# Chunyu-Hugh/SymbolicRegression.jl

Measured on AMD Instinct MI355X. Metric: tree-node x row evals/sec (batched eval_loss, fp32), higher is better.
Workload: dtype f32

## Files before the change

symbolicregression.jl_amd/csrc/sr_capi.cpp:

```cpp
#include <hip/hip_runtime.h>
#include <rccl/rccl.h>
#include <dlfcn.h>
#include <limits.h>
#include <stdlib.h>

#include <algorithm>
#include <atomic>
#include <chrono>
#include <cmath>
#include <cstdio>
#include <cstdlib>
#include <cstring>
#include <deque>
#include <functional>
#include <memory>
#include <mutex>
#include <string>
#include <vector>

#include "../../include/sr_amd.h"
#include "sr_compile.h"
#include "sr_eval.h"
#include "sr_fold.h"
#include "sr_fold_dev.h"
// ... 206 lines not shown
  DevBuf stamps;
  int64_t n_stamps = 0;
#endif
  std::unique_ptr<SrComm> xport;
  int comm_ranks = 0;
  int comm_rank = 0;
  uint64_t comm_gen = 0;
  DevBuf coll_buf, coll_packed, ctl;
  HostBuf h_coll;
  double last_eval_ms = 0.0, last_total_ms = 0.0;
  double last_busy_ms = 0.0;
  bool timing_pending = false;
  double phase_ms[5] = {0, 0, 0, 0, 0};
  std::chrono::steady_clock::time_point phase_t;
  void start_phases(std::chrono::steady_clock::time_point t) {
    phase_t = t;
    for (double& v : phase_ms) v = 0.0;
  }
  void mark_phase(int i) {
    const auto now = std::chrono::steady_clock::now();
    phase_ms[i] = std::chrono::duration<double, std::milli>(now - phase_t).count();
    phase_t = now;
  }
  int cu_count = 256;
  std::vector<uint32_t> perm_host;
  DevBuf fold_cand;
  DevBuf fold_list;
  DevBuf fold_wg;
  DevBuf loss_list;
  DevBuf fold_est;
  DevBuf fold_dbg;
  DevBuf fold_code, fold_tab, fold_store, fold_ctl, fold_io2, fold_sq, fold_tab2;
  std::shared_ptr<void> fold_job;
  size_t outs_fval_off = 0, outs_fst_off = 0, outs_bytes_all = 0;
  hipEvent_t ev_fc0[kMaxChunks] = {}, ev_fc1[kMaxChunks] = {};
  int64_t n_ref_ok_last = 0, n_ref_fail_last = 0;
  double fold_kernel_ms_last = 0.0;
// ... 297 lines not shown

template <typename T>
struct BatchCall {
  sr_ctx* ctx;
  const EvalReq& req;
  const BatchWants& want;
  SrProgramBatch<T>* prog;
  BatchResult* res;
  sr_ctx::LastCall scratch;
  sr_ctx::LastCall& last;
  bool allow_derived;
  BatchCall(sr_ctx* c, const EvalReq& q, const BatchWants& w, SrProgramBatch<T>* p, BatchResult* r)
      : ctx(c), req(q), want(w), prog(p), res(r), last(w.internal ? scratch : c->last), allow_derived(w.allow_derived) {}
  void mark_phase(int i) {
    if (!want.internal) ctx->mark_phase(i);
  }
  bool gather = false, multi = false;
  int64_t n_eval = 0, n_rows_up = 0, nt = 0, total_nodes = 0;
  int mrb = 0, lkind = 0;
  double lparam = 0.0;
  const sr_ctx::LossExpr* lexpr = nullptr;
  const sr_param_batch* pb = nullptr;
  bool parametric = false;
  int nfk = 0;
  int64_t p_stride = 0;
  double max_abs_p = 0.0;
  int tier = 0, R = 0, W = 0, Rv = 0, n_rb = 1, n_chunks = 1;
  SrBuildRequest breq;
  GridSpec gs;
  Grid g_ls, g_vs;
// ... 117 lines not shown
    img = sr_prog_image(total_nodes, nt, sizeof(SrIns<T>), multi ? size_t(req.views->n_views) : 0);
    SR_HIP_CHECK(ctx->prog.ensure(img.bytes));
    SR_HIP_CHECK(ctx->h_prog.ensure(img.bytes, s, ctx->stream2));
    dprog = ctx->prog.as<char>();
    ctx->d_code = dprog;
    ctx->d_off = reinterpret_cast<uint32_t*>(dprog + img.o_off);
    ctx->d_bad = reinterpret_cast<uint8_t*>(dprog + img.o_bad);
    ctx->d_perm = reinterpret_cast<uint32_t*>(dprog + img.o_perm);
    ctx->d_end = reinterpret_cast<uint32_t*>(dprog + img.o_end);
    n_part = size_t(nt) * size_t(n_rb);
    SR_HIP_CHECK(ctx->part_sum.ensure(n_part * sizeof(double) + 8));
    SR_HIP_CHECK(ctx->part_flag.ensure(n_part * sizeof(uint32_t) + 4));
    return SR_OK;
  }

  int plan_fold() {
    fold_n_terms = want.shard ? ((req.ds->w && req.ds->shard_w_min < 0.0) ? 0 : want.n_total)
                              : fold_terms(req.ds, n_eval, req.loss_kind);
    if (want.shard) ctx->fold_job.reset();
    if (want.fold && ctx->ref_fold && want.mode == SR_MODE_LOSS && nt > 0 && fold_n_terms > 0) {
      FoldPlanIn in;
      in.nt = nt;
      in.n_eval = n_eval;
      in.max_shard = want.shard ? sr_max_shard_rows(req.ds->shard_offs, n_eval) : n_eval;
      in.fold_len = want.shard ? want.n_total : n_eval;
      in.elem_size = int(sizeof(T));
      in.tier = tier;
      in.R = R;
      in.Rv = Rv;
      in.fold_store_mb = ctx->fold_store_mb;
      in.fold_slot_mb = ctx->fold_slot_mb;
      in.fold_seg_max = ctx->fold_seg_max;
      in.fold_rows_max = ctx->fold_rows_max;
      in.g_ls = g_ls;
      in.g_vs = g_vs;
      in.g_big = gs.over(in.max_shard, std::max<int64_t>(512, (in.max_shard + ctx->fold_seg_max - 1) /
                                                                     std::max<int64_t>(1, ctx->fold_seg_max)))
                     .grid(nt, R, 1);
      fold = sr_fold_plan(in);
      if (fold.path == 1) {
        SR_HIP_CHECK(ctx->fold_store.ensure(size_t(nt) * size_t(fold.pos_rows) * sizeof(T)));
      } else if (fold.path == 2) {
        SR_HIP_CHECK(ctx->fold_store.ensure(size_t(fold.slots) * size_t(fold.slot_rows) * sizeof(T)));
        SR_HIP_CHECK(ctx->fold_ctl.ensure(64));
        SR_HIP_CHECK(hipMemsetAsync(ctx->fold_ctl.p, 0, 4 * sizeof(int), s));
      }
      if (fold.path && ctx->fold_stats) {
        SR_HIP_CHECK(ctx->fold_dbg.ensure(size_t(nt) * sizeof(int4) + 16));
        SR_HIP_CHECK(hipMemsetAsync(ctx->fold_dbg.p, 0, size_t(nt) * sizeof(int4), s));
      }
      if (fold.path) {
        SR_HIP_CHECK(ctx->fold_code.ensure(n_part * sizeof(int32_t) + 4));
        SR_HIP_CHECK(ctx->fold_tab.ensure(n_part * sizeof(typename SrFoldTab<T>::Pair) + 16));
        SR_HIP_CHECK(ctx->fold_sq.ensure(n_part * sizeof(int32_t) + 4));
        SR_HIP_CHECK(ctx->fold_tab2.ensure(n_part * sizeof(typename SrFoldTab<T>::Pair) + 16));
      }
    }
    fold_cand = fold.path == 2 && ctx->fold_single_pass && sizeof(T) == 4 && tier == SR_TIER_BASIC && !gather &&
                !multi && !want.shard && !parametric && n_rb > 1;
    if (fold_cand) SR_HIP_CHECK(ctx->fold_cand.ensure(n_part * sizeof(int4) + 16));
    if (fold_cand && ctx->fold_cand_est) {
      SR_HIP_CHECK(ctx->fold_est.ensure(size_t(nt) * (sizeof(double) + sizeof(uint32_t)) + 8));
      SR_HIP_CHECK(hipMemsetAsync(ctx->fold_est.p, 0, size_t(nt) * (sizeof(double) + sizeof(uint32_t)), s));
    }
    fold_compact = fold.path == 2 && ctx->fold_compact && !gather && !multi && !want.shard && !parametric;
    if (fold_compact) {
      SR_HIP_CHECK(ctx->fold_list.ensure(n_part * sizeof(int32_t) + 4));
      SR_HIP_CHECK(ctx->fold_wg.ensure(sr_fold_wg_words(n_rb) * sizeof(int32_t)));
    }
    loss_compact = fold_compact && fold_cand && ctx->loss_compact && want.mode == SR_MODE_LOSS;
    if (loss_compact) SR_HIP_CHECK(ctx->loss_list.ensure(sr_loss_list_bytes(nt)));
    for (int c = 0; c < kMaxChunks; ++c) last.loss_listed_np[c] = 0;
    last.loss_list_nt = nt;
    last.loss_list_read = true;
    last.n_loss_listed_launches = last.n_loss_live = last.n_loss_excl = 0;
    for (int r = 0; r < 2 * kMaxChunks; ++r) {
      last.fold_wg_nrb[r] = 0;
      for (int k = 0; k < 4; ++k) last.fold_wg_info[r][k] = 0.0;
    }
    last.fold_wg_read = true;
    last.fold_path = res->fold_path = fold.path;
    last.fold_timed = false;
    last.fold_cand_read = fold.path != 2;
    last.n_cand_taken = last.n_cand_rerun = 0;
    return SR_OK;
// ... 103 lines not shown
    ctx->h_perm_last = h_perm;
    h_end = reinterpret_cast<uint32_t*>(hprog + img.o_end);
    last.n_chunks = 0;
    last.derived = false;
    last.n_derived = 0;
    last.timed = ctx->timing != 0 && !want.internal;
    if (last.timed) SR_HIP_CHECK(hipEventRecord(ctx->ev_start, s));
    if (gather)
      SR_HIP_CHECK(hipMemcpyAsync(ctx->row_idx.p, req.row_idx, size_t(n_rows_up) * sizeof(int64_t), hipMemcpyHostToDevice,
                                  s));
    if (parametric && nt > 0 && p_stride > 0)
      SR_HIP_CHECK(hipMemcpyAsync(ctx->ptab.p, ctx->h_ptab.p, size_t(nt) * size_t(p_stride) * sizeof(T), hipMemcpyHostToDevice, s));
    return SR_OK;
  }

  int launch_derived() {
    dld = (n_eval + kRowAlign - 1) / kRowAlign * kRowAlign;
    max_abs_x = leaf_bound(want.shard ? want.shard->max_abs_x : req.ds->max_abs_x);
    const int64_t derived_rows = want.shard ? want.shard->min_rows : n_eval;
    if (allow_derived && ctx->derived && want.mode == SR_MODE_LOSS && tier == SR_TIER_BASIC &&
        derived_rows >= kDerivedMinRows && nt >= 64 && double(nt) * double(derived_rows) >= kDerivedMinWork &&
        max_abs_x < double(tbig())) {
      choose_derived(*req.trees, ctx->opsets[req.opset_id], req.ds->nf, &spec, &dmap);
      if (spec.n > 0) {
        SR_HIP_CHECK(ctx->derived_cols.ensure(size_t(spec.n) * size_t(dld) * sizeof(T)));
        if (last.timed) SR_HIP_CHECK(hipEventRecord(ctx->ev_d0, s));
        SR_HIP_CHECK(sr_launch_derived<T>(static_cast<const T*>(req.ds->X), req.ds->ld,
                                          gather ? ctx->row_idx.as<int64_t>() : nullptr, n_eval, dld, spec,
                                          ctx->derived_cols.as<T>(), dld, s));
        if (last.timed) SR_HIP_CHECK(hipEventRecord(ctx->ev_d1, s));
        last.derived = true;
        last.n_derived = spec.n;
      } else {
        dmap.clear();
      }
    }
    stress_probe = use_probe && !gather && req.ds->probe_rows != nullptr && ctx->stress_probe;
    if (stress_probe && !dmap.empty()) {
      SR_HIP_CHECK(ctx->probe_derived.ensure(size_t(spec.n) * size_t(kProbeRows) * sizeof(T)));
      SR_HIP_CHECK(sr_launch_derived<T>(static_cast<const T*>(req.ds->X), req.ds->ld,
                                        static_cast<const int64_t*>(req.ds->probe_rows), req.ds->n_probe, kProbeRows, spec,
                                        ctx->probe_derived.as<T>(), kProbeRows, s));
    }
    return SR_OK;
  }

  int begin_chunks() {
    if (n_chunks > 1) {
      SR_HIP_CHECK(ctx->need_stream2());
      SR_HIP_CHECK(hipEventRecord(ctx->ev_join, s));
// ... 7 lines not shown
    fjob.slot_rows = fold.slot_rows;
    fjob.n_terms = fold_n_terms;
    fjob.delta = std::ldexp(1.0, -ctx->fold_delta_log2);
    fjob.fuse_reduce = fold.path == 1 && !want.shard && want.mode == SR_MODE_LOSS;
    fjob.slot_cap = fold.path == 2
                        ? int(std::min<int64_t>({int64_t(INT_MAX / 2), fold.slot_budget,
                                                 int64_t(ctx->fold_store.cap / (size_t(fold.slot_rows) * sizeof(T)))}))
                        : 0;
    char* const outs_base = (host_out || fold_mirror) ? ctx->h_outs.as<char>() : ctx->outs.as<char>();
    d_fval = reinterpret_cast<T*>(outs_base + ctx->outs_fval_off);
    d_fst = reinterpret_cast<int32_t*>(outs_base + ctx->outs_fst_off);
    t_pre = std::chrono::steady_clock::now();
    return SR_OK;
  }

  int compile_chunk(BatchChunk<T>& ch) {
    static const bool phase_debug = std::getenv("SR_AMD_PHASE_DEBUG") != nullptr;
    const int64_t t0 = ch.t0 = cplan.bound[ch.c];
    const int64_t nc = ch.nc = cplan.bound[ch.c + 1] - t0;
    for (int64_t t = t0; t < t0 + nc; ++t)
      ch.max_nodes = std::max<uint32_t>(ch.max_nodes, uint32_t(req.trees->offsets[t + 1] - req.trees->offsets[t]));
    ch.cs = (ch.c & 1) ? ctx->stream2 : s;
    sr_tree_batch sub = *req.trees;
    sub.n_trees = nc;
    sub.offsets = req.trees->offsets + t0;
    ch.pc.keep_pieces = true;
    const SrParamNodes pnodes{parametric ? pb->is_parameter : nullptr, parametric ? pb->parameter : nullptr,
                              parametric ? pb->max_parameters : 0};
    const int rc = sr_compile_batch<T>(sub, ctx->opsets[req.opset_id], want.n_total, req.ds->nf, false, &ch.pc, &err,
                                       dmap.empty() ? nullptr : dmap.data(), parametric ? &pnodes : nullptr);
    if (rc != SR_OK) {
      if (rc == SR_ERR_BAD_TREE || rc == SR_ERR_INVALID_ARG) {
        const size_t at = err.find("tree ");
        if (at == 0) {
          const int64_t k = std::atoll(err.c_str() + 5);
          err = "tree " + std::to_string(k + t0) + err.substr(err.find(':'));
        }
      }
      return set_error(rc, err);
    }
    if (ch.c == 0) {
      if (phase_debug) {
        const auto now = std::chrono::steady_clock::now();
        std::fprintf(stderr, "[sr phase] trees %lld chunks %d: setup %.3f ms, compile of chunk 0 (%lld trees) %.3f ms\n",
                     (long long)nt, n_chunks, std::chrono::duration<double, std::milli>(t_pre - ctx->phase_t).count(),
                     (long long)nc, std::chrono::duration<double, std::milli>(now - t_pre).count());
      }
      mark_phase(0);
    }
    ch.depth = ch.pc.max_depth > 0 ? ch.pc.max_depth : 1;
    ch.ncode = ch.pc.n_code;
    return SR_OK;
  }

  int order_and_stage(BatchChunk<T>& ch) {
    const SrProgramBatch<T>& pc = ch.pc;
    const int64_t t0 = ch.t0, nc = ch.nc;
    ch.n_vs = sr_count_vstk(pc.depth.data(), nc, Rv > 0);
    if (ch.n_vs > 0) ch.g_vs = gs.grid(ch.n_vs, Rv, 0);
// ... 240 lines not shown
      who.mflag = reinterpret_cast<uint32_t*>(ctx->h_outs.as<char>() + ctx->outs_flag_off);
    }
    for (const FoldRegion<T>& fr : fjob.regions) {
      SR_STAGE(fold_steps<T>(ctx, fjob, fr, who, cs));
      SR_STAGE(fold_walk<T>(ctx, fjob, fr, who, nullptr, d_fval, d_fst, cs));
    }
    fjob.regions.clear();
    if (last.timed) {
      SR_HIP_CHECK(hipEventRecord(ctx->ev_fc1[ch.c], cs));
      last.fold_timed = true;
    }
    return SR_OK;
  }

  int run_chunk(int c) {
    BatchChunk<T> ch;
    ch.c = c;
    SR_STAGE(compile_chunk(ch));
    SR_STAGE(order_and_stage(ch));
    SR_STAGE(upload_chunk(ch));
    if (last.timed) SR_HIP_CHECK(hipEventRecord(ctx->ev_c0[c], ch.cs));
    if (ch.n_vs > 0) SR_STAGE(launch_region(ch, 0, ch.n_vs, true));
    if (ch.n_vs < ch.nc) SR_STAGE(launch_region(ch, ch.n_vs, ch.nc - ch.n_vs, false));
    if (last.timed) SR_HIP_CHECK(hipEventRecord(ctx->ev_c1[c], ch.cs));
    if (early) SR_HIP_CHECK(hipEventRecord(ctx->ev_red[c], ch.cs));
    if (early && c == n_chunks - 1) {
      for (int k = 0; k < c; ++k) SR_HIP_CHECK(hipStreamWaitEvent(ch.cs, ctx->ev_red[k], 0));
      SR_HIP_CHECK(hipMemcpyAsync(ctx->h_outs.as<char>() + ctx->outs_flag_off, ctx->outs.as<char>() + ctx->outs_flag_off,
                                  size_t(nt) * sizeof(uint32_t), hipMemcpyDeviceToHost, ch.cs));
      SR_HIP_CHECK(hipEventRecord(ctx->ev_flags, ch.cs));
    }
    if (fold.path && !want.shard && !fjob.regions.empty()) SR_STAGE(fold_chunk(ch));
    last.n_chunks = c + 1;
    code_base += uint32_t(ch.ncode);
    return SR_OK;
  }

  int run() {
    SR_STAGE(validate_call());
    SR_STAGE(stage_param_table());
    choose_kernels();
    SR_STAGE(bind_buffers());
    in_flight = true;
    SR_STAGE(plan_fold());
    SR_STAGE(plan_chunks());
    SR_STAGE(bind_outputs());
    SR_STAGE(prepare_hints());
    SR_STAGE(begin_programs());
    SR_STAGE(launch_derived());
    SR_STAGE(begin_chunks());
    for (int c = 0; c < n_chunks && nt > 0; ++c) SR_STAGE(run_chunk(c));
    if (n_chunks > 1) {
      SR_HIP_CHECK(hipEventRecord(ctx->ev_join, ctx->stream2));
      SR_HIP_CHECK(hipStreamWaitEvent(s, ctx->ev_join, 0));
    }
    if (nt == 0) mark_phase(0);
    res->grid = glast;
    if (fold.path && want.shard) ctx->fold_job = std::make_shared<FoldJob<T>>(std::move(fjob));
    mark_phase(1);
    return SR_OK;
  }
};

template <typename T>
// ... 765 lines not shown
        float km = 0.f;
        if (hipEventElapsedTime(&km, ctx->ev_k0, ctx->ev_k1) == hipSuccess) ctx->exact_kernel_ms += double(km);
      }
      exact_done = one_batch || mc == 0;
      return SR_OK;
    }();
    if (rc != SR_OK) {
      (void)hipStreamSynchronize(s);
      if (ctx->stream2) (void)hipStreamSynchronize(ctx->stream2);
      if (ctx->stream3) (void)hipStreamSynchronize(ctx->stream3);
      return rc;
    }
  } else {
    SR_HIP_CHECK(hipStreamSynchronize(s));
  }
  if (!ctx->host_reductions.empty()) host_reduce_partials(ctx, nt);
  std::vector<double> sums(hs, hs + nt);
  std::vector<uint32_t> flags(hf, hf + nt);
  ctx->timing_pending = true;
  if (!c.res.early) {
    ctx->mark_phase(2);
    big_list(flags.data(), &list);
    list_ok.assign(list.size(), 1);
    ctx->n_exact_last = int64_t(list.size());
    ctx->exact_kernel_ms = 0.0;
  }
  for (int v = 0; v < n_views && !list.empty() && !exact_done; ++v) {
    std::vector<int64_t> lv;
    std::vector<size_t> at;
    for (size_t i = 0; i < list.size(); ++i)
// ... 62 lines not shown
  ctx->n_fold_last = int64_t(fold_list.size());
  ctx->fold_slow_last = ctx->fold_seg_last = 0;
  for (double& v : ctx->fold_ms) v = 0.0;
  for (int v = 0; v < n_views && !fold_list.empty(); ++v) {
    std::vector<int64_t> fv;
    for (int64_t t : fold_list)
      if (view_of(t) == v) fv.push_back(t);
    if (fv.empty()) continue;
    std::vector<T> fold;
    rc = fold_exact<T>(ctx, q.view(v), n_eval, fv, &fold);
    if (rc != SR_OK) return rc;
    const T den = (ds->w && n_eval > 0) ? jl_wsum_view<T>(ds, rows_of(v), n_eval) : T(vden[size_t(v)]);
    for (size_t i = 0; i < fv.size(); ++i) static_cast<T*>(c.out_loss)[fv[i]] = T(fold[i] / den);
  }
  ctx->mark_phase(4);
  auto t1 = std::chrono::steady_clock::now();
  ctx->last_total_ms = std::chrono::duration<double, std::milli>(t1 - c.t0).count();
  return SR_OK;
}

template <typename T>
int eval_loss_impl(sr_ctx* ctx, const EvalReq& req, void* out_loss, uint8_t* out_complete) {
  LossCall<T> c;
  const int rc = eval_loss_submit<T>(ctx, req, out_loss, out_complete, &c);
  if (rc != SR_OK) return rc;
  return eval_loss_finish<T>(ctx, c);
}

template <typename T>
int eval_pred_impl(sr_ctx* ctx, const EvalReq& req, void* out_pred, uint8_t* out_complete) {
// ... 2102 lines not shown
      int64_t entries = 0, longest = 0;
      for (int b = 0; b < nrb; ++b) {
        entries += cnt[b];
        longest = std::max<int64_t>(longest, cnt[b]);
      }
      ctx->last.fold_wg_info[r][0] = double(wg0[nrb]);
      ctx->last.fold_wg_info[r][1] = double(entries);
      ctx->last.fold_wg_info[r][2] = double(wg0[nrb + 1]);
      ctx->last.fold_wg_info[r][3] = double(longest);
    }
    ctx->last.fold_wg_read = true;
  }
  for (int r = 0; r < 2 * kMaxChunks; ++r)
    for (int k = 0; k < 4; ++k)
      if (n > 19 + 4 * r + k) out[19 + 4 * r + k] = ctx->last.fold_wg_info[r][k];
  return SR_OK;
}

int sr_set_tuning(sr_ctx* ctx, const char* name, int64_t value) {
  if (check_ctx(ctx) != SR_OK) return SR_ERR_INVALID_ARG;
  if (!name) return set_error(SR_ERR_INVALID_ARG, "tuning knob name is NULL");
  Lock l(ctx);
  std::string err;
  return sr_knob_set(*ctx, name, value, &err) == 0 ? SR_OK : set_error(SR_ERR_INVALID_ARG, err);
}

int sr_last_grad_info(sr_ctx* ctx, int n, double* kernel_ms, double* flops, int64_t* items, int* rows_per_lane) {
  if (check_ctx(ctx) != SR_OK) return SR_ERR_INVALID_ARG;
  Lock l(ctx);
  for (int b = 0; b < n && b < sr_ctx::kGradBuckets; ++b) {
// ... 69 lines not shown
```

symbolicregression.jl_amd/csrc/sr_compile.cpp:

```cpp
#include "sr_compile.h"

#include <unistd.h>

#include <algorithm>
#include <atomic>
#include <chrono>
#include <cstdlib>
#include <cmath>
#include <condition_variable>
#include <cstring>
#include <functional>
#include <mutex>
#include <thread>

namespace {

class WorkerPool {
 public:
  static WorkerPool& get() {
    static std::mutex m;
    static WorkerPool* pool = nullptr;
    std::lock_guard<std::mutex> g(m);
    if (!pool || pool->pid_ != getpid()) pool = new WorkerPool();
    return *pool;
  }
  int size() const { return int(threads_.size()) + 1; }
  void run(int n, const std::function<void(int)>& fn) {
    std::lock_guard<std::mutex> batch(batch_mu_);
    uint64_t g;
    {
      std::lock_guard<std::mutex> lk(mu_);
      g = ++gen_;
      job_ = &fn;
      n_jobs_ = n;
      done_.store(0);
      ticket_.store(g << 32);
      gen_pub_.store(g, std::memory_order_release);
    }
    if (n > 1 && !threads_.empty()) cv_.notify_all();
    drain(g, &fn, n);
    while (done_.load(std::memory_order_acquire) < n) std::this_thread::yield();
  }

 private:
  WorkerPool() : pid_(getpid()) {
    unsigned hc = std::thread::hardware_concurrency();
    int n = int(hc == 0 ? 4 : (hc > 16 ? 16 : hc));
    if (const char* v = std::getenv("SR_AMD_COMPILE_THREADS")) n = std::atoi(v) > 0 ? std::atoi(v) : 1;
    if (const char* v = std::getenv("SR_AMD_COMPILE_SPIN_US")) spin_us_ = std::max(0, std::atoi(v));
    --n;
    for (int i = 0; i < n; ++i) threads_.emplace_back([this] { loop(); });
    for (auto& t : threads_) t.detach();
  }
  void drain(uint64_t g, const std::function<void(int)>* job, int n) {
    uint64_t t = ticket_.load();
    for (;;) {
      if ((t >> 32) != g || int(t & 0xffffffffu) >= n) return;
      if (!ticket_.compare_exchange_weak(t, t + 1)) continue;
      (*job)(int(t & 0xffffffffu));
      done_.fetch_add(1, std::memory_order_release);
      t = ticket_.load();
    }
  }
  void loop() {
    uint64_t seen = 0;
    for (;;) {
      uint64_t g;
      const std::function<void(int)>* job;
      int n;
      const auto t0 = std::chrono::steady_clock::now();
      while (gen_pub_.load(std::memory_order_acquire) == seen &&
             std::chrono::steady_clock::now() - t0 < std::chrono::microseconds(spin_us_))
        std::this_thread::yield();
      {
        std::unique_lock<std::mutex> lk(mu_);
        cv_.wait(lk, [&] { return gen_ != seen; });
        seen = g = gen_;
        job = job_;
        n = n_jobs_;
      }
      drain(g, job, n);
    }
  }
  pid_t pid_;
  std::vector<std::thread> threads_;
  std::mutex batch_mu_, mu_;
  std::condition_variable cv_;
  const std::function<void(int)>* job_ = nullptr;
  int n_jobs_ = 0;
  std::atomic<uint64_t> ticket_{0};
  std::atomic<int> done_{0};
  uint64_t gen_ = 0;
  std::atomic<uint64_t> gen_pub_{0};
  int spin_us_ = 0;
};

struct NameId {
  const char* name;
  uint32_t id;
};

const NameId kUnary[] = {
    {"neg", SR_U_NEG},       {"-", SR_U_NEG},          {"square", SR_U_SQUARE},  {"cube", SR_U_CUBE},
    {"exp", SR_U_EXP},       {"cos", SR_U_COS},        {"sin", SR_U_SIN},        {"tan", SR_U_TAN},
    {"log", SR_U_LOG},       {"safe_log", SR_U_LOG},   {"log2", SR_U_LOG2},      {"safe_log2", SR_U_LOG2},
    {"log10", SR_U_LOG10},   {"safe_log10", SR_U_LOG10}, {"log1p", SR_U_LOG1P}, {"safe_log1p", SR_U_LOG1P},
    {"sqrt", SR_U_SQRT},     {"safe_sqrt", SR_U_SQRT}, {"abs", SR_U_ABS},        {"sign", SR_U_SIGN},
    {"tanh", SR_U_TANH},     {"sinh", SR_U_SINH},      {"cosh", SR_U_COSH},      {"atan", SR_U_ATAN},
    {"asin", SR_U_ASIN},     {"safe_asin", SR_U_ASIN}, {"acos", SR_U_ACOS},      {"safe_acos", SR_U_ACOS},
    {"acosh", SR_U_ACOSH},   {"safe_acosh", SR_U_ACOSH}, {"atanh", SR_U_ATANH}, {"safe_atanh", SR_U_ATANH},
// ... 575 lines not shown
  for (const auto& e : kUnary)
    if (std::strcmp(e.name, name) == 0) return e.id;
  return 0;
}
uint32_t sr_binary_id(const char* name) {
  for (const auto& e : kBinary)
    if (std::strcmp(e.name, name) == 0) return e.id;
  return 0;
}

void sr_parallel_for(int n, const std::function<void(int)>& fn) {
  if (n <= 1) {
    if (n == 1) fn(0);
    return;
  }
  WorkerPool::get().run(n, fn);
}

template <typename T>
int sr_compile_batch(const sr_tree_batch& trees, const SrOpset& ops, int64_t n_rows, int64_t nfeatures,
                     bool with_const_index, SrProgramBatch<T>* out, std::string* err, const int16_t* derived,
                     const SrParamNodes* pn) {
  const int64_t nt = trees.n_trees;
  if (pn && nt > 0 && (!pn->is_parameter || !pn->parameter || pn->max_parameters < 0)) {
    *err = "sr_param_batch has NULL arrays";
    return SR_ERR_INVALID_ARG;
  }
  if (nt < 0 || (nt > 0 && (!trees.offsets || !trees.degree || !trees.op || !trees.feature ||
                            !trees.constant || !trees.val))) {
    *err = "sr_tree_batch has NULL arrays";
    return SR_ERR_INVALID_ARG;
  }
  struct PerTree {
    int thread;
    uint32_t begin, len;
    uint8_t bad;
    uint32_t checks, consts, cost;
    int depth;
    int64_t nodes, ops;
  };
  std::vector<PerTree> per(size_t(nt > 0 ? nt : 0));
  std::vector<int> errs(size_t(nt > 0 ? nt : 0), SR_OK);
  const T* vals = static_cast<const T*>(trees.val);
  const int64_t pool = nt > 128 ? WorkerPool::get().size() : 1;
  static const int64_t min_piece = [] {
    const char* v = std::getenv("SR_AMD_COMPILE_PIECE");
    return v ? std::max<int64_t>(1, std::atoll(v)) : int64_t(32);
  }();
  const int64_t kPiece = std::max<int64_t>(min_piece, std::min<int64_t>(256, (nt + 4 * pool - 1) / (4 * pool)));
  const int n_pieces = int(nt <= kPiece ? 1 : (nt + kPiece - 1) / kPiece);
  const int nthreads = n_pieces;
  std::vector<std::vector<SrIns<T>>> bufs(static_cast<size_t>(nthreads));

  auto work = [&](int w, int64_t lo, int64_t hi) {
    TreeCompiler<T> tc(ops, n_rows, nfeatures, with_const_index, with_const_index ? nullptr : derived);
    if (pn) tc.max_params = pn->max_parameters;
    std::vector<SrIns<T>>& buf = bufs[size_t(w)];
    buf.reserve(size_t(trees.offsets[hi] - trees.offsets[lo]));
    for (int64_t k = lo; k < hi; ++k) {
      const int64_t b = trees.offsets[k], e = trees.offsets[k + 1];
      if (e < b) {
        errs[k] = SR_ERR_BAD_TREE;
        continue;
      }
      Tree<T> tree;
      tree.degree = trees.degree + b;
      tree.op = trees.op + b;
      tree.feature = trees.feature + b;
      tree.constant = trees.constant + b;
      tree.val = vals + b;
// ... 11 lines not shown
      for (const auto& in : tc.code) cost += sr_instruction_cost(in.op);
      PerTree& p = per[k];
      p.thread = w;
      p.begin = uint32_t(buf.size());
      p.len = uint32_t(tc.code.size());
      buf.insert(buf.end(), tc.code.begin(), tc.code.end());
      p.cost = cost;
      p.bad = (tc.bad || tc.code.empty()) ? 1 : 0;
      p.checks = tc.n_checks;
      p.consts = tc.n_consts;
      p.depth = tc.max_depth;
      p.nodes = e - b;
      p.ops = 0;
      for (int64_t i = b; i < e; ++i) p.ops += trees.degree[i] > 0 ? 1 : 0;
    }
  };
  if (n_pieces <= 1) {
    work(0, 0, nt);
  } else {
    WorkerPool::get().run(n_pieces, [&](int w) {
      const int64_t lo = int64_t(w) * kPiece, hi = (lo + kPiece < nt) ? lo + kPiece : nt;
      if (lo < hi) work(w, lo, hi);
    });
  }
  for (int64_t k = 0; k < nt; ++k)
    if (errs[k] != SR_OK) {
      *err = "tree " + std::to_string(k) + ": malformed tree or operator index";
      return errs[k];
    }
  out->code.clear();
  out->offsets.assign(size_t(nt + 1), 0);
  out->static_bad.assign(size_t(nt), 0);
  out->n_checks.assign(size_t(nt), 0);
  out->n_consts.assign(size_t(nt), 0);
  out->const_off.assign(size_t(nt + 1), 0);
  out->cost.assign(size_t(nt), 0);
  out->depth.assign(size_t(nt), 0);
  out->max_depth = 0;
  out->max_checks = 0;
  out->total_nodes = 0;
  out->total_ops = 0;
  size_t total = 0;
  for (int64_t k = 0; k < nt; ++k) total += per[k].len;
  out->n_code = total;
  const bool lazy = out->keep_pieces;
  if (lazy) {
    out->piece.resize(size_t(nt));
    out->begin.resize(size_t(nt));
  } else {
    out->code.resize(total);
  }
  size_t at = 0;
  for (int64_t k = 0; k < nt; ++k) {
    const PerTree& p = per[k];
    out->offsets[k] = uint32_t(at);
    if (lazy) {
      out->piece[size_t(k)] = uint32_t(p.thread);
      out->begin[size_t(k)] = p.begin;
    } else if (p.len) {
      std::memcpy(out->code.data() + at, bufs[size_t(p.thread)].data() + p.begin, size_t(p.len) * sizeof(SrIns<T>));
    }
    at += p.len;
    out->static_bad[k] = p.bad;
    out->cost[k] = p.bad ? 0u : p.cost;
    out->depth[k] = uint8_t(p.bad ? 0 : (p.depth > 255 ? 255 : p.depth));
    out->n_checks[k] = p.checks;
    out->n_consts[k] = p.consts;
    out->const_off[k + 1] = out->const_off[k] + p.consts;
    if (p.depth > out->max_depth) out->max_depth = p.depth;
    if (int(p.checks) > out->max_checks) out->max_checks = int(p.checks);
    out->total_nodes += p.nodes;
    out->total_ops += p.ops;
  }
  out->offsets[nt] = uint32_t(total);
  if (lazy) out->pieces = std::move(bufs);
  return SR_OK;
}

template int sr_compile_batch<float>(const sr_tree_batch&, const SrOpset&, int64_t, int64_t, bool,
                                     SrProgramBatch<float>*, std::string*, const int16_t*, const SrParamNodes*);
template int sr_compile_batch<double>(const sr_tree_batch&, const SrOpset&, int64_t, int64_t, bool,
                                      SrProgramBatch<double>*, std::string*, const int16_t*, const SrParamNodes*);
```

symbolicregression.jl_amd/csrc/sr_compile.h:

```cpp
#pragma once
#include <stdint.h>
#include <functional>
#include <string>
#include <vector>
#include "sr_ops.h"
#include "../../include/sr_amd.h"

struct SrOpset {
  std::vector<uint32_t> unary;
  std::vector<uint32_t> binary;
};

uint32_t sr_unary_id(const char* name);
uint32_t sr_binary_id(const char* name);

template <typename T>
struct SrProgramBatch {
  std::vector<SrIns<T>> code;
  std::vector<uint32_t> offsets;
  std::vector<uint8_t> static_bad;
  std::vector<uint32_t> n_checks;
  std::vector<uint32_t> n_consts;
  std::vector<uint32_t> const_off;
  std::vector<uint32_t> cost;
// ... 13 lines not shown
};

void sr_parallel_for(int n, const std::function<void(int)>& fn);

uint32_t sr_instruction_cost(uint32_t opcode);

struct SrParamNodes {
  const uint8_t* is_parameter;
  const uint16_t* parameter;
  int32_t max_parameters;
};
template <typename T>
int sr_compile_batch(const sr_tree_batch& trees, const SrOpset& ops, int64_t n_rows, int64_t nfeatures,
                     bool with_const_index, SrProgramBatch<T>* out, std::string* err,
                     const int16_t* derived = nullptr, const SrParamNodes* pn = nullptr);
```

Baseline: 32090 billion.

## Overlap chunk-0 tree compilation on worker pool with host setup

Splits tree compilation into an asynchronous start/finish job so the first chunk's compile runs on pool threads while the main thread binds buffers, plans fold and launches derived columns. The fold decisions and derived-column choice are moved ahead of compilation because compilation needs the derived map. The worker pool is extracted into a shared header with separate start/finish and an abandon path. It also adds per-call timing marks. The aim is to hide host compile latency behind setup work. In exchange the pool's batch lock is held across stages, which adds concurrency complexity.

After: 32230 billion (median of 4 runs). About the same (+0.4%).

```diff
diff --git a/symbolicregression.jl_amd/csrc/sr_capi.cpp b/symbolicregression.jl_amd/csrc/sr_capi.cpp
--- a/symbolicregression.jl_amd/csrc/sr_capi.cpp
+++ b/symbolicregression.jl_amd/csrc/sr_capi.cpp
@@ -244,13 +244,20 @@
   double phase_ms[5] = {0, 0, 0, 0, 0};
   std::chrono::steady_clock::time_point phase_t;
   void start_phases(std::chrono::steady_clock::time_point t) {
-    phase_t = t;
+    phase_t = call_t0 = t;
     for (double& v : phase_ms) v = 0.0;
+    for (double& v : call_ms) v = 0.0;
   }
   void mark_phase(int i) {
     const auto now = std::chrono::steady_clock::now();
     phase_ms[i] = std::chrono::duration<double, std::milli>(now - phase_t).count();
     phase_t = now;
+  }
+  enum { kCallChosen = 0, kCallDerived, kCallCompiled, kCallStaged, kCallUploaded, kCallLaunched, kCallSynced, kCallFinal, kCallMarks };
+  double call_ms[kCallMarks] = {};
+  std::chrono::steady_clock::time_point call_t0;
+  void mark_call(int i) {
+    call_ms[i] = std::chrono::duration<double, std::milli>(std::chrono::steady_clock::now() - call_t0).count();
   }
   int cu_count = 256;
   std::vector<uint32_t> perm_host;
@@ -578,6 +585,9 @@
       : ctx(c), req(q), want(w), prog(p), res(r), last(w.internal ? scratch : c->last), allow_derived(w.allow_derived) {}
   void mark_phase(int i) {
     if (!want.internal) ctx->mark_phase(i);
+  }
+  void mark_call(int i) {
+    if (!want.internal) ctx->mark_call(i);
   }
   bool gather = false, multi = false;
   int64_t n_eval = 0, n_rows_up = 0, nt = 0, total_nodes = 0;
@@ -725,10 +735,9 @@
     return SR_OK;
   }
 
-  int plan_fold() {
+  void decide_fold() {
     fold_n_terms = want.shard ? ((req.ds->w && req.ds->shard_w_min < 0.0) ? 0 : want.n_total)
                               : fold_terms(req.ds, n_eval, req.loss_kind);
-    if (want.shard) ctx->fold_job.reset();
     if (want.fold && ctx->ref_fold && want.mode == SR_MODE_LOSS && nt > 0 && fold_n_terms > 0) {
       FoldPlanIn in;
       in.nt = nt;
@@ -749,6 +758,15 @@
                                                                      std::max<int64_t>(1, ctx->fold_seg_max)))
                      .grid(nt, R, 1);
       fold = sr_fold_plan(in);
+    }
+    fold_cand = fold.path == 2 && ctx->fold_single_pass && sizeof(T) == 4 && tier == SR_TIER_BASIC && !gather &&
+                !multi && !want.shard && !parametric && n_rb > 1;
+    fold_compact = fold.path == 2 && ctx->fold_compact && !gather && !multi && !want.shard && !parametric;
+    loss_compact = fold_compact && fold_cand && ctx->loss_compact && want.mode == SR_MODE_LOSS;
+  }
+  int plan_fold() {
+    if (want.shard) ctx->fold_job.reset();
+    if (fold.path) {
       if (fold.path == 1) {
         SR_HIP_CHECK(ctx->fold_store.ensure(size_t(nt) * size_t(fold.pos_rows) * sizeof(T)));
       } else if (fold.path == 2) {
@@ -767,19 +785,15 @@
         SR_HIP_CHECK(ctx->fold_tab2.ensure(n_part * sizeof(typename SrFoldTab<T>::Pair) + 16));
       }
     }
-    fold_cand = fold.path == 2 && ctx->fold_single_pass && sizeof(T) == 4 && tier == SR_TIER_BASIC && !gather &&
-                !multi && !want.shard && !parametric && n_rb > 1;
     if (fold_cand) SR_HIP_CHECK(ctx->fold_cand.ensure(n_part * sizeof(int4) + 16));
     if (fold_cand && ctx->fold_cand_est) {
       SR_HIP_CHECK(ctx->fold_est.ensure(size_t(nt) * (sizeof(double) + sizeof(uint32_t)) + 8));
       SR_HIP_CHECK(hipMemsetAsync(ctx->fold_est.p, 0, size_t(nt) * (sizeof(double) + sizeof(uint32_t)), s));
     }
-    fold_compact = fold.path == 2 && ctx->fold_compact && !gather && !multi && !want.shard && !parametric;
     if (fold_compact) {
       SR_HIP_CHECK(ctx->fold_list.ensure(n_part * sizeof(int32_t) + 4));
       SR_HIP_CHECK(ctx->fold_wg.ensure(sr_fold_wg_words(n_rb) * sizeof(int32_t)));
     }
-    loss_compact = fold_compact && fold_cand && ctx->loss_compact && want.mode == SR_MODE_LOSS;
     if (loss_compact) SR_HIP_CHECK(ctx->loss_list.ensure(sr_loss_list_bytes(nt)));
     for (int c = 0; c < kMaxChunks; ++c) last.loss_listed_np[c] = 0;
     last.loss_list_nt = nt;
@@ -913,7 +927,7 @@
     return SR_OK;
   }
 
-  int launch_derived() {
+  void choose_columns() {
     dld = (n_eval + kRowAlign - 1) / kRowAlign * kRowAlign;
     max_abs_x = leaf_bound(want.shard ? want.shard->max_abs_x : req.ds->max_abs_x);
     const int64_t derived_rows = want.shard ? want.shard->min_rows : n_eval;
@@ -921,18 +935,19 @@
         derived_rows >= kDerivedMinRows && nt >= 64 && double(nt) * double(derived_rows) >= kDerivedMinWork &&
         max_abs_x < double(tbig())) {
       choose_derived(*req.trees, ctx->opsets[req.opset_id], req.ds->nf, &spec, &dmap);
-      if (spec.n > 0) {
-        SR_HIP_CHECK(ctx->derived_cols.ensure(size_t(spec.n) * size_t(dld) * sizeof(T)));
-        if (last.timed) SR_HIP_CHECK(hipEventRecord(ctx->ev_d0, s));
-        SR_HIP_CHECK(sr_launch_derived<T>(static_cast<const T*>(req.ds->X), req.ds->ld,
-                                          gather ? ctx->row_idx.as<int64_t>() : nullptr, n_eval, dld, spec,
-                                          ctx->derived_cols.as<T>(), dld, s));
-        if (last.timed) SR_HIP_CHECK(hipEventRecord(ctx->ev_d1, s));
-        last.derived = true;
-        last.n_derived = spec.n;
-      } else {
-        dmap.clear();
-      }
+      if (spec.n <= 0) dmap.clear();
+    }
+  }
+  int launch_derived() {
+    if (!dmap.empty()) {
+      SR_HIP_CHECK(ctx->derived_cols.ensure(size_t(spec.n) * size_t(dld) * sizeof(T)));
+      if (last.timed) SR_HIP_CHECK(hipEventRecord(ctx->ev_d0, s));
+      SR_HIP_CHECK(sr_launch_derived<T>(static_cast<const T*>(req.ds->X), req.ds->ld,
+                                        gather ? ctx->row_idx.as<int64_t>() : nullptr, n_eval, dld, spec,
+                                        ctx->derived_cols.as<T>(), dld, s));
+      if (last.timed) SR_HIP_CHECK(hipEventRecord(ctx->ev_d1, s));
+      last.derived = true;
+      last.n_derived = spec.n;
     }
     stress_probe = use_probe && !gather && req.ds->probe_rows != nullptr && ctx->stress_probe;
     if (stress_probe && !dmap.empty()) {
@@ -970,21 +985,26 @@
     return SR_OK;
   }
 
-  int compile_chunk(BatchChunk<T>& ch) {
-    static const bool phase_debug = std::getenv("SR_AMD_PHASE_DEBUG") != nullptr;
+  int compile_start(BatchChunk<T>& ch, SrCompileJob<T>& job) {
     const int64_t t0 = ch.t0 = cplan.bound[ch.c];
     const int64_t nc = ch.nc = cplan.bound[ch.c + 1] - t0;
     for (int64_t t = t0; t < t0 + nc; ++t)
       ch.max_nodes = std::max<uint32_t>(ch.max_nodes, uint32_t(req.trees->offsets[t + 1] - req.trees->offsets[t]));
-    ch.cs = (ch.c & 1) ? ctx->stream2 : s;
     sr_tree_batch sub = *req.trees;
     sub.n_trees = nc;
     sub.offsets = req.trees->offsets + t0;
     ch.pc.keep_pieces = true;
     const SrParamNodes pnodes{parametric ? pb->is_parameter : nullptr, parametric ? pb->parameter : nullptr,
                               parametric ? pb->max_parameters : 0};
-    const int rc = sr_compile_batch<T>(sub, ctx->opsets[req.opset_id], want.n_total, req.ds->nf, false, &ch.pc, &err,
-                                       dmap.empty() ? nullptr : dmap.data(), parametric ? &pnodes : nullptr);
+    const int rc = job.start(sub, ctx->opsets[req.opset_id], want.n_total, req.ds->nf, false, &ch.pc, &err,
+                             dmap.empty() ? nullptr : dmap.data(), parametric ? &pnodes : nullptr);
+    return rc != SR_OK ? set_error(rc, err) : SR_OK;
+  }
+  int compile_finish(BatchChunk<T>& ch, SrCompileJob<T>& job) {
+    static const bool phase_debug = std::getenv("SR_AMD_PHASE_DEBUG") != nullptr;
+    const int64_t t0 = ch.t0, nc = ch.nc;
+    ch.cs = (ch.c & 1) ? ctx->stream2 : s;
+    const int rc = job.finish();
     if (rc != SR_OK) {
       if (rc == SR_ERR_BAD_TREE || rc == SR_ERR_INVALID_ARG) {
         const size_t at = err.find("tree ");
@@ -998,7 +1018,7 @@
     if (ch.c == 0) {
       if (phase_debug) {
         const auto now = std::chrono::steady_clock::now();
-        std::fprintf(stderr, "[sr phase] trees %lld chunks %d: setup %.3f ms, compile of chunk 0 (%lld trees) %.3f ms\n",
+        std::fprintf(stderr, "[sr phase] trees %lld chunks %d: setup %.3f ms (chunk 0's compile beside it), its join (%lld trees) %.3f ms\n",
                      (long long)nt, n_chunks, std::chrono::duration<double, std::milli>(t_pre - ctx->phase_t).count(),
                      (long long)nc, std::chrono::duration<double, std::milli>(now - t_pre).count());
       }
@@ -1269,13 +1289,21 @@
   }
 
   int run_chunk(int c) {
-    BatchChunk<T> ch;
-    ch.c = c;
-    SR_STAGE(compile_chunk(ch));
+    BatchChunk<T> later;
+    BatchChunk<T>& ch = c == 0 ? first : later;
+    if (!job.started()) {
+      ch.c = c;
+      SR_STAGE(compile_start(ch, job));
+    }
+    SR_STAGE(compile_finish(ch, job));
+    if (c == 0) mark_call(sr_ctx::kCallCompiled);
     SR_STAGE(order_and_stage(ch));
+    if (c == 0) mark_call(sr_ctx::kCallStaged);
     SR_STAGE(upload_chunk(ch));
+    if (c == 0) mark_call(sr_ctx::kCallUploaded);
     if (last.timed) SR_HIP_CHECK(hipEventRecord(ctx->ev_c0[c], ch.cs));
     if (ch.n_vs > 0) SR_STAGE(launch_region(ch, 0, ch.n_vs, true));
+    if (c == 0) mark_call(sr_ctx::kCallLaunched);
     if (ch.n_vs < ch.nc) SR_STAGE(launch_region(ch, ch.n_vs, ch.nc - ch.n_vs, false));
     if (last.timed) SR_HIP_CHECK(hipEventRecord(ctx->ev_c1[c], ch.cs));
     if (early) SR_HIP_CHECK(hipEventRecord(ctx->ev_red[c], ch.cs));
@@ -1291,18 +1319,36 @@
     return SR_OK;
   }
 
+  BatchChunk<T> first;
+  SrCompileJob<T> job;
+  int start_first_compile() {
+    first.c = 0;
+    return nt > 0 && n_chunks > 1 ? compile_start(first, job) : SR_OK;
+  }
+  void leave_compile() { job.abandon(); }
+
   int run() {
+    const int rc = run_stages();
+    leave_compile();
+    return rc;
+  }
+  int run_stages() {
     SR_STAGE(validate_call());
     SR_STAGE(stage_param_table());
     choose_kernels();
+    mark_call(sr_ctx::kCallChosen);
+    decide_fold();
+    SR_STAGE(plan_chunks());
+    choose_columns();
+    SR_STAGE(start_first_compile());
     SR_STAGE(bind_buffers());
     in_flight = true;
     SR_STAGE(plan_fold());
-    SR_STAGE(plan_chunks());
     SR_STAGE(bind_outputs());
     SR_STAGE(prepare_hints());
     SR_STAGE(begin_programs());
     SR_STAGE(launch_derived());
+    mark_call(sr_ctx::kCallDerived);
     SR_STAGE(begin_chunks());
     for (int c = 0; c < n_chunks && nt > 0; ++c) SR_STAGE(run_chunk(c));
     if (n_chunks > 1) {
@@ -2098,6 +2144,7 @@
   } else {
     SR_HIP_CHECK(hipStreamSynchronize(s));
   }
+  ctx->mark_call(sr_ctx::kCallSynced);
   if (!ctx->host_reductions.empty()) host_reduce_partials(ctx, nt);
   std::vector<double> sums(hs, hs + nt);
   std::vector<uint32_t> flags(hf, hf + nt);
@@ -2190,6 +2237,7 @@
     for (size_t i = 0; i < fv.size(); ++i) static_cast<T*>(c.out_loss)[fv[i]] = T(fold[i] / den);
   }
   ctx->mark_phase(4);
+  ctx->mark_call(sr_ctx::kCallFinal);
   auto t1 = std::chrono::steady_clock::now();
   ctx->last_total_ms = std::chrono::duration<double, std::milli>(t1 - c.t0).count();
   return SR_OK;
@@ -4322,6 +4370,8 @@
   for (int r = 0; r < 2 * kMaxChunks; ++r)
     for (int k = 0; k < 4; ++k)
       if (n > 19 + 4 * r + k) out[19 + 4 * r + k] = ctx->last.fold_wg_info[r][k];
+  for (int i = 0; i < sr_ctx::kCallMarks; ++i)
+    if (n > 51 + i) out[51 + i] = ctx->call_ms[i];
   return SR_OK;
 }
 
diff --git a/symbolicregression.jl_amd/csrc/sr_compile.cpp b/symbolicregression.jl_amd/csrc/sr_compile.cpp
--- a/symbolicregression.jl_amd/csrc/sr_compile.cpp
+++ b/symbolicregression.jl_amd/csrc/sr_compile.cpp
@@ -1,4 +1,5 @@
 #include "sr_compile.h"
+#include "sr_pool.h"
 
 #include <unistd.h>
 
@@ -14,86 +15,6 @@
 #include <thread>
 
 namespace {
-
-class WorkerPool {
- public:
-  static WorkerPool& get() {
-    static std::mutex m;
-    static WorkerPool* pool = nullptr;
-    std::lock_guard<std::mutex> g(m);
-    if (!pool || pool->pid_ != getpid()) pool = new WorkerPool();
-    return *pool;
-  }
-  int size() const { return int(threads_.size()) + 1; }
-  void run(int n, const std::function<void(int)>& fn) {
-    std::lock_guard<std::mutex> batch(batch_mu_);
-    uint64_t g;
-    {
-      std::lock_guard<std::mutex> lk(mu_);
-      g = ++gen_;
-      job_ = &fn;
-      n_jobs_ = n;
-      done_.store(0);
-      ticket_.store(g << 32);
-      gen_pub_.store(g, std::memory_order_release);
-    }
-    if (n > 1 && !threads_.empty()) cv_.notify_all();
-    drain(g, &fn, n);
-    while (done_.load(std::memory_order_acquire) < n) std::this_thread::yield();
-  }
-
- private:
-  WorkerPool() : pid_(getpid()) {
-    unsigned hc = std::thread::hardware_concurrency();
-    int n = int(hc == 0 ? 4 : (hc > 16 ? 16 : hc));
-    if (const char* v = std::getenv("SR_AMD_COMPILE_THREADS")) n = std::atoi(v) > 0 ? std::atoi(v) : 1;
-    if (const char* v = std::getenv("SR_AMD_COMPILE_SPIN_US")) spin_us_ = std::max(0, std::atoi(v));
-    --n;
-    for (int i = 0; i < n; ++i) threads_.emplace_back([this] { loop(); });
-    for (auto& t : threads_) t.detach();
-  }
-  void drain(uint64_t g, const std::function<void(int)>* job, int n) {
-    uint64_t t = ticket_.load();
-    for (;;) {
-      if ((t >> 32) != g || int(t & 0xffffffffu) >= n) return;
-      if (!ticket_.compare_exchange_weak(t, t + 1)) continue;
-      (*job)(int(t & 0xffffffffu));
-      done_.fetch_add(1, std::memory_order_release);
-      t = ticket_.load();
-    }
-  }
-  void loop() {
-    uint64_t seen = 0;
-    for (;;) {
-      uint64_t g;
-      const std::function<void(int)>* job;
-      int n;
-      const auto t0 = std::chrono::steady_clock::now();
-      while (gen_pub_.load(std::memory_order_acquire) == seen &&
-             std::chrono::steady_clock::now() - t0 < std::chrono::microseconds(spin_us_))
-        std::this_thread::yield();
-      {
-        std::unique_lock<std::mutex> lk(mu_);
-        cv_.wait(lk, [&] { return gen_ != seen; });
-        seen = g = gen_;
-        job = job_;
-        n = n_jobs_;
-      }
-      drain(g, job, n);
-    }
-  }
-  pid_t pid_;
-  std::vector<std::thread> threads_;
-  std::mutex batch_mu_, mu_;
-  std::condition_variable cv_;
-  const std::function<void(int)>* job_ = nullptr;
-  int n_jobs_ = 0;
-  std::atomic<uint64_t> ticket_{0};
-  std::atomic<int> done_{0};
-  uint64_t gen_ = 0;
-  std::atomic<uint64_t> gen_pub_{0};
-  int spin_us_ = 0;
-};
 
 struct NameId {
   const char* name;
@@ -699,23 +620,11 @@
     if (n == 1) fn(0);
     return;
   }
-  WorkerPool::get().run(n, fn);
-}
-
-template <typename T>
-int sr_compile_batch(const sr_tree_batch& trees, const SrOpset& ops, int64_t n_rows, int64_t nfeatures,
-                     bool with_const_index, SrProgramBatch<T>* out, std::string* err, const int16_t* derived,
-                     const SrParamNodes* pn) {
-  const int64_t nt = trees.n_trees;
-  if (pn && nt > 0 && (!pn->is_parameter || !pn->parameter || pn->max_parameters < 0)) {
-    *err = "sr_param_batch has NULL arrays";
-    return SR_ERR_INVALID_ARG;
-  }
-  if (nt < 0 || (nt > 0 && (!trees.offsets || !trees.degree || !trees.op || !trees.feature ||
-                            !trees.constant || !trees.val))) {
-    *err = "sr_tree_batch has NULL arrays";
-    return SR_ERR_INVALID_ARG;
-  }
+  SrWorkerPool::get().run(n, fn);
+}
+
+template <typename T>
+struct SrCompileJob<T>::Impl {
   struct PerTree {
     int thread;
     uint32_t begin, len;
@@ -724,21 +633,26 @@
     int depth;
     int64_t nodes, ops;
   };
-  std::vector<PerTree> per(size_t(nt > 0 ? nt : 0));
-  std::vector<int> errs(size_t(nt > 0 ? nt : 0), SR_OK);
-  const T* vals = static_cast<const T*>(trees.val);
-  const int64_t pool = nt > 128 ? WorkerPool::get().size() : 1;
-  static const int64_t min_piece = [] {
-    const char* v = std::getenv("SR_AMD_COMPILE_PIECE");
-    return v ? std::max<int64_t>(1, std::atoll(v)) : int64_t(32);
-  }();
-  const int64_t kPiece = std::max<int64_t>(min_piece, std::min<int64_t>(256, (nt + 4 * pool - 1) / (4 * pool)));
-  const int n_pieces = int(nt <= kPiece ? 1 : (nt + kPiece - 1) / kPiece);
-  const int nthreads = n_pieces;
-  std::vector<std::vector<SrIns<T>>> bufs(static_cast<size_t>(nthreads));
-
-  auto work = [&](int w, int64_t lo, int64_t hi) {
-    TreeCompiler<T> tc(ops, n_rows, nfeatures, with_const_index, with_const_index ? nullptr : derived);
+  sr_tree_batch trees{};
+  const SrOpset* ops = nullptr;
+  int64_t n_rows = 0, nfeatures = 0;
+  bool with_const_index = false;
+  SrProgramBatch<T>* out = nullptr;
+  std::string* err = nullptr;
+  const int16_t* derived = nullptr;
+  SrParamNodes pnodes{};
+  const SrParamNodes* pn = nullptr;
+  std::vector<PerTree> per;
+  std::vector<int> errs;
+  std::vector<std::vector<SrIns<T>>> bufs;
+  int64_t kPiece = 1;
+  int n_pieces = 0;
+  std::function<void(int)> piece_fn;
+  bool started = false, pooled = false;
+
+  void work(int w, int64_t lo, int64_t hi) {
+    const T* vals = static_cast<const T*>(trees.val);
+    TreeCompiler<T> tc(*ops, n_rows, nfeatures, with_const_index, with_const_index ? nullptr : derived);
     if (pn) tc.max_params = pn->max_parameters;
     std::vector<SrIns<T>>& buf = bufs[size_t(w)];
     buf.reserve(size_t(trees.offsets[hi] - trees.offsets[lo]));
@@ -780,67 +694,156 @@
       p.ops = 0;
       for (int64_t i = b; i < e; ++i) p.ops += trees.degree[i] > 0 ? 1 : 0;
     }
-  };
-  if (n_pieces <= 1) {
-    work(0, 0, nt);
-  } else {
-    WorkerPool::get().run(n_pieces, [&](int w) {
-      const int64_t lo = int64_t(w) * kPiece, hi = (lo + kPiece < nt) ? lo + kPiece : nt;
-      if (lo < hi) work(w, lo, hi);
-    });
-  }
-  for (int64_t k = 0; k < nt; ++k)
-    if (errs[k] != SR_OK) {
-      *err = "tree " + std::to_string(k) + ": malformed tree or operator index";
-      return errs[k];
-    }
-  out->code.clear();
-  out->offsets.assign(size_t(nt + 1), 0);
-  out->static_bad.assign(size_t(nt), 0);
-  out->n_checks.assign(size_t(nt), 0);
-  out->n_consts.assign(size_t(nt), 0);
-  out->const_off.assign(size_t(nt + 1), 0);
-  out->cost.assign(size_t(nt), 0);
-  out->depth.assign(size_t(nt), 0);
-  out->max_depth = 0;
-  out->max_checks = 0;
-  out->total_nodes = 0;
-  out->total_ops = 0;
-  size_t total = 0;
-  for (int64_t k = 0; k < nt; ++k) total += per[k].len;
-  out->n_code = total;
-  const bool lazy = out->keep_pieces;
-  if (lazy) {
-    out->piece.resize(size_t(nt));
-    out->begin.resize(size_t(nt));
-  } else {
-    out->code.resize(total);
-  }
-  size_t at = 0;
-  for (int64_t k = 0; k < nt; ++k) {
-    const PerTree& p = per[k];
-    out->offsets[k] = uint32_t(at);
+  }
+
+  int start() {
+    const int64_t nt = trees.n_trees;
+    if (pn && nt > 0 && (!pn->is_parameter || !pn->parameter || pn->max_parameters < 0)) {
+      *err = "sr_param_batch has NULL arrays";
+      return SR_ERR_INVALID_ARG;
+    }
+    if (nt < 0 || (nt > 0 && (!trees.offsets || !trees.degree || !trees.op || !trees.feature ||
+                              !trees.constant || !trees.val))) {
+      *err = "sr_tree_batch has NULL arrays";
+      return SR_ERR_INVALID_ARG;
+    }
+    per.assign(size_t(nt > 0 ? nt : 0), PerTree{});
+    errs.assign(size_t(nt > 0 ? nt : 0), SR_OK);
+    const int64_t pool = nt > 128 ? SrWorkerPool::get().size() : 1;
+    static const int64_t min_piece = [] {
+      const char* v = std::getenv("SR_AMD_COMPILE_PIECE");
+      return v ? std::max<int64_t>(1, std::atoll(v)) : int64_t(32);
+    }();
+    kPiece = std::max<int64_t>(min_piece, std::min<int64_t>(256, (nt + 4 * pool - 1) / (4 * pool)));
+    n_pieces = int(nt <= kPiece ? 1 : (nt + kPiece - 1) / kPiece);
+    bufs.assign(static_cast<size_t>(n_pieces), {});
+    started = true;
+    pooled = n_pieces > 1;
+    if (pooled) {
+      piece_fn = [this](int w) {
+        const int64_t n = trees.n_trees;
+        const int64_t lo = int64_t(w) * kPiece, hi = (lo + kPiece < n) ? lo + kPiece : n;
+        if (lo < hi) work(w, lo, hi);
+      };
+      SrWorkerPool::get().start(n_pieces, piece_fn);
+    }
+    return SR_OK;
+  }
+
+  void abandon() {
+    if (started && pooled) SrWorkerPool::get().finish(false);
+    started = pooled = false;
+  }
+
+  int finish() {
+    const int64_t nt = trees.n_trees;
+    if (pooled) SrWorkerPool::get().finish();
+    else work(0, 0, nt);
+    started = pooled = false;
+    for (int64_t k = 0; k < nt; ++k)
+      if (errs[k] != SR_OK) {
+        *err = "tree " + std::to_string(k) + ": malformed tree or operator index";
+        return errs[k];
+      }
+    out->code.clear();
+    out->offsets.assign(size_t(nt + 1), 0);
+    out->static_bad.assign(size_t(nt), 0);
+    out->n_checks.assign(size_t(nt), 0);
+    out->n_consts.assign(size_t(nt), 0);
+    out->const_off.assign(size_t(nt + 1), 0);
+    out->cost.assign(size_t(nt), 0);
+    out->depth.assign(size_t(nt), 0);
+    out->max_depth = 0;
+    out->max_checks = 0;
+    out->total_nodes = 0;
+    out->total_ops = 0;
+    size_t total = 0;
+    for (int64_t k = 0; k < nt; ++k) total += per[k].len;
+    out->n_code = total;
+    const bool lazy = out->keep_pieces;
     if (lazy) {
-      out->piece[size_t(k)] = uint32_t(p.thread);
-      out->begin[size_t(k)] = p.begin;
-    } else if (p.len) {
-      std::memcpy(out->code.data() + at, bufs[size_t(p.thread)].data() + p.begin, size_t(p.len) * sizeof(SrIns<T>));
-    }
-    at += p.len;
-    out->static_bad[k] = p.bad;
-    out->cost[k] = p.bad ? 0u : p.cost;
-    out->depth[k] = uint8_t(p.bad ? 0 : (p.depth > 255 ? 255 : p.depth));
-    out->n_checks[k] = p.checks;
-    out->n_consts[k] = p.consts;
-    out->const_off[k + 1] = out->const_off[k] + p.consts;
-    if (p.depth > out->max_depth) out->max_depth = p.depth;
-    if (int(p.checks) > out->max_checks) out->max_checks = int(p.checks);
-    out->total_nodes += p.nodes;
-    out->total_ops += p.ops;
-  }
-  out->offsets[nt] = uint32_t(total);
-  if (lazy) out->pieces = std::move(bufs);
-  return SR_OK;
+      out->piece.resize(size_t(nt));
+      out->begin.resize(size_t(nt));
+    } else {
+      out->code.resize(total);
+    }
+    size_t at = 0;
+    for (int64_t k = 0; k < nt; ++k) {
+      const PerTree& p = per[k];
+      out->offsets[k] = uint32_t(at);
+      if (lazy) {
+        out->piece[size_t(k)] = uint32_t(p.thread);
+        out->begin[size_t(k)] = p.begin;
+      } else if (p.len) {
+        std::memcpy(out->code.data() + at, bufs[size_t(p.thread)].data() + p.begin, size_t(p.len) * sizeof(SrIns<T>));
+      }
+      at += p.len;
+      out->static_bad[k] = p.bad;
+      out->cost[k] = p.bad ? 0u : p.cost;
+      out->depth[k] = uint8_t(p.bad ? 0 : (p.depth > 255 ? 255 : p.depth));
+      out->n_checks[k] = p.checks;
+      out->n_consts[k] = p.consts;
+      out->const_off[k + 1] = out->const_off[k] + p.consts;
+      if (p.depth > out->max_depth) out->max_depth = p.depth;
+      if (int(p.checks) > out->max_checks) out->max_checks = int(p.checks);
+      out->total_nodes += p.nodes;
+      out->total_ops += p.ops;
+    }
+    out->offsets[nt] = uint32_t(total);
+    if (lazy) out->pieces = std::move(bufs);
+    return SR_OK;
+  }
+};
+
+template <typename T>
+SrCompileJob<T>::SrCompileJob() : p_(new Impl()) {}
+template <typename T>
+SrCompileJob<T>::~SrCompileJob() {
+  p_->abandon();
+  delete p_;
+}
+template <typename T>
+bool SrCompileJob<T>::started() const {
+  return p_->started;
+}
+template <typename T>
+int SrCompileJob<T>::start(const sr_tree_batch& trees, const SrOpset& ops, int64_t n_rows, int64_t nfeatures,
+                           bool with_const_index, SrProgramBatch<T>* out, std::string* err, const int16_t* derived,
+                           const SrParamNodes* pn) {
+  p_->abandon();
+  p_->trees = trees;
+  p_->ops = &ops;
+  p_->n_rows = n_rows;
+  p_->nfeatures = nfeatures;
+  p_->with_const_index = with_const_index;
+  p_->out = out;
+  p_->err = err;
+  p_->derived = derived;
+  p_->pn = nullptr;
+  if (pn) {
+    p_->pnodes = *pn;
+    p_->pn = &p_->pnodes;
+  }
+  return p_->start();
+}
+template <typename T>
+int SrCompileJob<T>::finish() {
+  return p_->finish();
+}
+template <typename T>
+void SrCompileJob<T>::abandon() {
+  p_->abandon();
+}
+template class SrCompileJob<float>;
+template class SrCompileJob<double>;
+
+template <typename T>
+int sr_compile_batch(const sr_tree_batch& trees, const SrOpset& ops, int64_t n_rows, int64_t nfeatures,
+                     bool with_const_index, SrProgramBatch<T>* out, std::string* err, const int16_t* derived,
+                     const SrParamNodes* pn) {
+  SrCompileJob<T> job;
+  const int rc = job.start(trees, ops, n_rows, nfeatures, with_const_index, out, err, derived, pn);
+  return rc != SR_OK ? rc : job.finish();
 }
 
 template int sr_compile_batch<float>(const sr_tree_batch&, const SrOpset&, int64_t, int64_t, bool,
diff --git a/symbolicregression.jl_amd/csrc/sr_compile.h b/symbolicregression.jl_amd/csrc/sr_compile.h
--- a/symbolicregression.jl_amd/csrc/sr_compile.h
+++ b/symbolicregression.jl_amd/csrc/sr_compile.h
@@ -51,3 +51,21 @@
 int sr_compile_batch(const sr_tree_batch& trees, const SrOpset& ops, int64_t n_rows, int64_t nfeatures,
                      bool with_const_index, SrProgramBatch<T>* out, std::string* err,
                      const int16_t* derived = nullptr, const SrParamNodes* pn = nullptr);
+
+template <typename T>
+class SrCompileJob {
+ public:
+  SrCompileJob();
+  ~SrCompileJob();
+  SrCompileJob(const SrCompileJob&) = delete;
+  SrCompileJob& operator=(const SrCompileJob&) = delete;
+  int start(const sr_tree_batch& trees, const SrOpset& ops, int64_t n_rows, int64_t nfeatures, bool with_const_index,
+            SrProgramBatch<T>* out, std::string* err, const int16_t* derived = nullptr, const SrParamNodes* pn = nullptr);
+  int finish();
+  void abandon();
+  bool started() const;
+
+ private:
+  struct Impl;
+  Impl* p_;
+};
diff --git a/symbolicregression.jl_amd/csrc/sr_pool.h b/symbolicregression.jl_amd/csrc/sr_pool.h
--- /dev/null
+++ b/symbolicregression.jl_amd/csrc/sr_pool.h
@@ -0,0 +1,108 @@
+#pragma once
+#include <unistd.h>
+
+#include <atomic>
+#include <chrono>
+#include <condition_variable>
+#include <cstdint>
+#include <cstdlib>
+#include <functional>
+#include <mutex>
+#include <thread>
+#include <vector>
+
+class SrWorkerPool {
+ public:
+  static SrWorkerPool& get() {
+    static std::mutex m;
+    static SrWorkerPool* pool = nullptr;
+    std::lock_guard<std::mutex> g(m);
+    if (!pool || pool->pid_ != getpid()) pool = new SrWorkerPool();
+    return *pool;
+  }
+  int size() const { return int(threads_.size()) + 1; }
+  void run(int n, const std::function<void(int)>& fn) {
+    start(n, fn);
+    finish();
+  }
+  void start(int n, const std::function<void(int)>& fn) {
+    batch_mu_.lock();
+    {
+      std::lock_guard<std::mutex> lk(mu_);
+      cur_gen_ = ++gen_;
+      job_ = &fn;
+      n_jobs_ = n;
+      done_.store(0);
+      ticket_.store(cur_gen_ << 32);
+      gen_pub_.store(cur_gen_, std::memory_order_release);
+    }
+    if (n > 1 && !threads_.empty()) cv_.notify_all();
+  }
+  void finish(bool run_rest = true) {
+    const uint64_t g = cur_gen_;
+    const int n = n_jobs_;
+    if (run_rest) {
+      drain(g, job_, n);
+    } else {
+      uint64_t t = ticket_.load();
+      while ((t >> 32) == g && int(t & 0xffffffffu) < n && !ticket_.compare_exchange_weak(t, (g << 32) | uint64_t(uint32_t(n)))) {
+      }
+      if ((t >> 32) == g && int(t & 0xffffffffu) < n) done_.fetch_add(n - int(t & 0xffffffffu), std::memory_order_release);
+    }
+    while (done_.load(std::memory_order_acquire) < n) std::this_thread::yield();
+    batch_mu_.unlock();
+  }
+
+ private:
+  SrWorkerPool() : pid_(getpid()) {
+    unsigned hc = std::thread::hardware_concurrency();
+    int n = int(hc == 0 ? 4 : (hc > 16 ? 16 : hc));
+    if (const char* v = std::getenv("SR_AMD_COMPILE_THREADS")) n = std::atoi(v) > 0 ? std::atoi(v) : 1;
+    if (const char* v = std::getenv("SR_AMD_COMPILE_SPIN_US")) spin_us_ = std::atoi(v) > 0 ? std::atoi(v) : 0;
+    --n;
+    for (int i = 0; i < n; ++i) threads_.emplace_back([this] { loop(); });
+    for (auto& t : threads_) t.detach();
+  }
+  void drain(uint64_t g, const std::function<void(int)>* job, int n) {
+    uint64_t t = ticket_.load();
+    for (;;) {
+      if ((t >> 32) != g || int(t & 0xffffffffu) >= n) return;
+      if (!ticket_.compare_exchange_weak(t, t + 1)) continue;
+      (*job)(int(t & 0xffffffffu));
+      done_.fetch_add(1, std::memory_order_release);
+      t = ticket_.load();
+    }
+  }
+  void loop() {
+    uint64_t seen = 0;
+    for (;;) {
+      uint64_t g;
+      const std::function<void(int)>* job;
+      int n;
+      const auto t0 = std::chrono::steady_clock::now();
+      while (gen_pub_.load(std::memory_order_acquire) == seen &&
+             std::chrono::steady_clock::now() - t0 < std::chrono::microseconds(spin_us_))
+        std::this_thread::yield();
+      {
+        std::unique_lock<std::mutex> lk(mu_);
+        cv_.wait(lk, [&] { return gen_ != seen; });
+        seen = g = gen_;
+        job = job_;
+        n = n_jobs_;
+      }
+      drain(g, job, n);
+    }
+  }
+  pid_t pid_;
+  std::vector<std::thread> threads_;
+  std::mutex batch_mu_, mu_;
+  std::condition_variable cv_;
+  const std::function<void(int)>* job_ = nullptr;
+  int n_jobs_ = 0;
+  std::atomic<uint64_t> ticket_{0};
+  std::atomic<int> done_{0};
+  uint64_t gen_ = 0;
+  uint64_t cur_gen_ = 0;
+  std::atomic<uint64_t> gen_pub_{0};
+  int spin_us_ = 0;
+};
```
